# aiven/tiered-storage-for-apache-kafka

Hardware: AMD Instinct MI355X
Metric: GiB/s segment chunk transform (Zstd+AES+CRC), 4MiB chunks (higher is better)
Workload: dtype u8

## Files before the change

### tiered-storage-for-apache-kafka_amd/csrc/crc_dev.h

```cpp
#pragma once
#include "tsx_internal.h"

#define POLY 0x82F63B78u

__host__ __device__ static inline uint32_t crc_mulx(uint32_t v) { return (v >> 1) ^ (POLY & (0u - (v & 1u))); }

__host__ __device__ static inline uint32_t crc_mulmod(uint32_t a, uint32_t b) {
    uint32_t acc = 0;
    for (int i = 0; i < 32; i++) {
        acc ^= b & (0u - ((a >> (31 - i)) & 1u));
        b = crc_mulx(b);
    }
    return acc;
}

__device__ static inline uint32_t crc_pow_pieces(const tsx_crc_tables* tab, uint32_t e) {
    uint32_t r = 0x80000000u;
    for (int k = 0; e; k++, e >>= 1)
        if (e & 1u) r = crc_mulmod(r, tab->pow2[k]);
    return r;
}


__device__ static inline uint32_t crc32c_wave(const tsx_crc_tables* __restrict__ tab, const uint8_t* __restrict__ buf, uint32_t len,
                                              uint32_t* ldsTab, uint32_t lane) {
    {
        const uint4* g = reinterpret_cast<const uint4*>(&tab->slice[0][0]);
        uint4* l = reinterpret_cast<uint4*>(ldsTab);
        for (uint32_t i = lane; i < 4 * 256 / 4; i += 64) l[i] = g[i];
    }
    __syncthreads();
    const uint32_t q = len >> 4;
    const uint32_t per = (((q + 63) >> 6) + 3) & ~3u;
    const uint32_t p0 = min(lane * per, q), p1 = min(p0 + per, q);
    const uint4* in = reinterpret_cast<const uint4*>(buf);
    uint32_t s = 0;
    #define CRC_W(x) { s ^= (x); s = ldsTab[3 * 256 + (s & 0xFF)] ^ ldsTab[2 * 256 + ((s >> 8) & 0xFF)] ^ ldsTab[256 + ((s >> 16) & 0xFF)] ^ ldsTab[s >> 24]; }
    uint32_t p = p0;
    if (p < p1 && p == 0) {
        const uint4 w = in[0];
        CRC_W(w.x ^ 0xFFFFFFFFu) CRC_W(w.y) CRC_W(w.z) CRC_W(w.w)
        p = 1;
    }
    for (; p + 4 <= p1; p += 4) {
        const uint4 w0 = in[p], w1 = in[p + 1], w2 = in[p + 2], w3 = in[p + 3];
        CRC_W(w0.x) CRC_W(w0.y) CRC_W(w0.z) CRC_W(w0.w)
        CRC_W(w1.x) CRC_W(w1.y) CRC_W(w1.z) CRC_W(w1.w)
        CRC_W(w2.x) CRC_W(w2.y) CRC_W(w2.z) CRC_W(w2.w)
        CRC_W(w3.x) CRC_W(w3.y) CRC_W(w3.z) CRC_W(w3.w)
    }
    for (; p < p1; p++) {
        const uint4 w = in[p];
        CRC_W(w.x) CRC_W(w.y) CRC_W(w.z) CRC_W(w.w)
    }
    #undef CRC_W
    uint32_t v = p1 > p0 ? crc_mulmod(s, crc_pow_pieces(tab, q - p1)) : 0u;
    for (int o = 32; o; o >>= 1) v ^= __shfl_xor(v, o);
    if (q == 0) v = 0xFFFFFFFFu;
    const uint8_t* t = buf + ((size_t)q << 4);
    for (uint32_t i = 0; i < (len & 15u); i++) {
        v ^= t[i];
        for (int k = 0; k < 8; k++) v = crc_mulx(v);
    }
    __syncthreads();
    return ~v;
}
```

### tiered-storage-for-apache-kafka_amd/csrc/zstd_enc.hip

```cpp
#include "zstd_common.h"
#ifdef ZS_DBG
#include <stdio.h>
#endif
#include "gcm_dev.h"
#include "crc_dev.h"
#include "svc_dev.h"
#define XXH_WAVE_ATTR __attribute__((noinline))
#include "xxh64_dev.h"

#define LANES 64
#define UNI(x) ((uint32_t)__builtin_amdgcn_readfirstlane((uint32_t)(x)))
#ifdef HIPEMU
#define ZS_GLOBAL
#else
#define ZS_GLOBAL __attribute__((address_space(1)))
#endif
typedef const ZS_GLOBAL uint8_t* gbytes_t;
typedef ZS_GLOBAL uint32_t* gwords_t;
struct __attribute__((packed)) zs_u64u { uint64_t v; };
struct __attribute__((packed)) zs_u32u { uint32_t v; };
__device__ static inline uint64_t gld64(gbytes_t p) { return reinterpret_cast<const ZS_GLOBAL zs_u64u*>(p)->v; }
__device__ static inline uint32_t gld32(gbytes_t p) { return reinterpret_cast<const ZS_GLOBAL zs_u32u*>(p)->v; }
__device__ static inline uint4 ld128a(const uint8_t* p) { return *reinterpret_cast<const uint4*>(p); }
#ifdef HIPEMU
// ... 101 lines not shown
            FseTable of;
            union {
                FseTable ml;
                uint32_t hist[256];
            };
            uint32_t hist2[256];
            uint8_t tableSymbol[512];
            uint16_t cumul[64];
            short norm[64];
        };
        struct {
            uint32_t ring[ZS_RING / 4 + 4];
            uint8_t scr[2 * ZS_SCR];
        } p;
        struct {
            tsx_gf128 tab[256];
            uint32_t t0[256];
        } g;
        uint32_t crcTab[4 * 256];
    };
};

#ifdef HIPEMU
#define WAVE_MEM_SYNC() __threadfence_block()
#define VM_DRAIN() do {} while (0)
#define LOADED64(x) do {} while (0)
#else
#define WAVE_MEM_SYNC() do { asm volatile("" ::: "memory"); __builtin_amdgcn_wave_barrier(); } while (0)
#define VM_DRAIN() asm volatile("s_waitcnt vmcnt(0)" ::: "memory")
#define LOADED64(x) do { uint32_t lo_ = (uint32_t)(x), hi_ = (uint32_t)((x) >> 32); asm volatile("" : "+v"(lo_), "+v"(hi_)); (x) = ((uint64_t)hi_ << 32) | lo_; } while (0)
#endif

struct Win { uint32_t lo, hi; };

__device__ static inline uint64_t ring8(const uint32_t* ring, uint32_t p) {
    uint64_t v; __builtin_memcpy(&v, reinterpret_cast<const uint8_t*>(ring) + (p & (ZS_RING - 1)), 8); return v;
}
__device__ static inline uint32_t ring4(const uint32_t* ring, uint32_t p) {
    uint32_t v; __builtin_memcpy(&v, reinterpret_cast<const uint8_t*>(ring) + (p & (ZS_RING - 1)), 4); return v;
}
__device__ static inline uint32_t ring1(const uint32_t* ring, uint32_t p) { return reinterpret_cast<const uint8_t*>(ring)[p & (ZS_RING - 1)]; }

template <class SP> __device__ __forceinline__ static void win_append(SP src, uint32_t lastPiece, uint32_t* ring, Win& w, uint32_t lane) {
    uint4 v[ZS_FILL / 1024];
    WAVE_MEM_SYNC();
#pragma unroll
    for (uint32_t k = 0; k < ZS_FILL / 1024; k++) {
        uint32_t pp = w.hi + k * 1024 + lane * 16;
        if (pp > lastPiece) pp = lastPiece;
        v[k] = ld128a(src + pp);
// ... 470 lines not shown
                            ip += rl; anchor = ip;
                        }
                    }
                    WAVE_MEM_SYNC();
                    break;
                }
                if (!validm || __builtin_amdgcn_readlane((uint32_t)inPair, 2 * np - 2) == 0) { evType = 4; break; }
                a = __builtin_amdgcn_readlane(la, 2 * np); an = __builtin_amdgcn_readlane(lan, 2 * np);
                s = __builtin_amdgcn_readlane(ls, 2 * np); ns = __builtin_amdgcn_readlane(lns, 2 * np);
                WAVE_MEM_SYNC();
                np = ZS_FAST_PAIRS;
            }
            if (evType == 4) break;
        }
    }
    sav2 = (sav1 != 0 && off1 != 0) ? sav1 : sav2;
    rep[0] = off1 ? off1 : sav1;
    rep[1] = off2 ? off2 : sav2;
    ms.nbSeq = nbSeq; ms.lastLL = iend - anchor; ms.anchor = anchor;
    ms.litSize = litSize + ms.lastLL;
#undef STORE_SEQ
}

__device__ static inline void copy_run(uint8_t* __restrict__ dst, const uint8_t* __restrict__ src, uint32_t n) {
    uint32_t k = 0;
    while (n - k >= 32) {
        const uint64_t a = ld64(src + k), b = ld64(src + k + 8), c = ld64(src + k + 16), d = ld64(src + k + 24);
        __builtin_memcpy(dst + k, &a, 8); __builtin_memcpy(dst + k + 8, &b, 8); __builtin_memcpy(dst + k + 16, &c, 8); __builtin_memcpy(dst + k + 24, &d, 8);
        k += 32;
    }
    const uint32_t r = n - k, nq = r >> 3;
    uint64_t q0 = 0, q1 = 0, q2 = 0; uint32_t w = 0; uint16_t h = 0; uint8_t b1 = 0;
    if (nq > 0) q0 = ld64(src + k);
    if (nq > 1) q1 = ld64(src + k + 8);
    if (nq > 2) q2 = ld64(src + k + 16);
    const uint32_t t = k + 8 * nq;
    if (r & 4) __builtin_memcpy(&w, src + t, 4);
    if (r & 2) __builtin_memcpy(&h, src + t + (r & 4), 2);
    if (r & 1) b1 = src[t + (r & 6)];
    if (nq > 0) __builtin_memcpy(dst + k, &q0, 8);
    if (nq > 1) __builtin_memcpy(dst + k + 8, &q1, 8);
    if (nq > 2) __builtin_memcpy(dst + k + 16, &q2, 8);
    if (r & 4) __builtin_memcpy(dst + t, &w, 4);
    if (r & 2) __builtin_memcpy(dst + t + (r & 4), &h, 2);
    if (r & 1) dst[t + (r & 6)] = b1;
}

__device__ ZS_NOINLINE static void gather_literals(uint8_t* __restrict__ lit, const uint8_t* __restrict__ src, const zs_seq* __restrict__ seqs,
                                                   uint32_t nbSeq, uint32_t tailPos, uint32_t tailLen, uint32_t lane) {
    uint32_t base = 0;
    for (uint32_t g = 0; g < nbSeq; g += LANES) {
        const uint32_t u = g + lane;
        uint32_t ll = 0, lp = 0;
        if (u < nbSeq) { const zs_seq q = seqs[u]; ll = q.litLength; lp = q.litPos; }
        uint32_t incl = ll;
        for (int o = 1; o < LANES; o <<= 1) { const uint32_t t = __shfl_up(incl, o); if (lane >= (uint32_t)o) incl += t; }
        const uint32_t dst = base + incl - ll;
        copy_run(lit + dst, src + lp, ll);
        base += __shfl(incl, LANES - 1);
    }
    for (uint32_t i = lane; i < tailLen; i += LANES) lit[base + i] = src[tailPos + i];
}

struct BitW { uint8_t* start; uint8_t* p; uint8_t* end; uint64_t acc; uint32_t n; bool overflow; };
__device__ static inline void bw_init(BitW& b, uint8_t* dst, uint8_t* end) { b.start = b.p = dst; b.end = end; b.acc = 0; b.n = 0; b.overflow = false; }
__device__ static inline void bw_add(BitW& b, uint64_t v, uint32_t nb) {
    if (!nb) return;
    b.acc |= (v & ((1ull << nb) - 1)) << b.n;
    b.n += nb;
    while (b.n >= 8) { if (b.p < b.end) *b.p++ = (uint8_t)b.acc; else b.overflow = true; b.acc >>= 8; b.n -= 8; }
}
__device__ static inline uint32_t bw_close(BitW& b) {
    bw_add(b, 1, 1);
    if (b.n) { if (b.p < b.end) *b.p++ = (uint8_t)b.acc; else b.overflow = true; b.n = 0; }
    return (uint32_t)(b.p - b.start);
}

__device__ static uint32_t fse_minTableLog(uint32_t srcSize, uint32_t maxSym) {
    uint32_t a = hb32(srcSize) + 1, b = hb32(maxSym) + 2;
    return a < b ? a : b;
}
__device__ static uint32_t fse_optimalTableLog(uint32_t maxTableLog, uint32_t srcSize, uint32_t maxSym, uint32_t minus) {
    uint32_t maxBitsSrc = hb32(srcSize - 1) - minus, tableLog = maxTableLog, minBits = fse_minTableLog(srcSize, maxSym);
    if (maxBitsSrc < tableLog) tableLog = maxBitsSrc;
// ... 430 lines not shown
                }
            }
        }
    }
    if ((hSize > 1) & (hSize < maxSym / 2)) { dst[0] = (uint8_t)hSize; return hSize + 1; }
    if (maxSym > 128) return 0xFFFFFFFFu;
    dst[0] = (uint8_t)(128 + (maxSym - 1));
    hw[maxSym] = 0;
    for (uint32_t n = 0; n < maxSym; n += 2) dst[(n / 2) + 1] = (uint8_t)((hw[n] << 4) + hw[n + 1]);
    return ((maxSym + 1) / 2) + 1;
}

__device__ static inline uint32_t wave_sum(uint32_t v) { for (int o = 32; o; o >>= 1) v += __shfl_xor(v, o); return v; }
__device__ static inline uint32_t wave_max(uint32_t v) { for (int o = 32; o; o >>= 1) { uint32_t t = __shfl_xor(v, o); v = t > v ? t : v; } return v; }
__device__ static inline uint32_t wave_excl_scan(uint32_t v, uint32_t lane) {
    uint32_t s = v;
    for (int o = 1; o < LANES; o <<= 1) { uint32_t t = __shfl_up(s, o); if (lane >= (uint32_t)o) s += t; }
    return s - v;
}

__device__ ZS_NOINLINE static void wave_histogram(uint32_t* hist, const uint8_t* __restrict__ p, uint32_t n, uint32_t lane) {
    for (uint32_t i = lane; i < 256; i += LANES) hist[i] = 0;
    __syncthreads();
    for (uint32_t i = lane; i < n; i += LANES) atomicAdd(&hist[p[i]], 1u);
    __syncthreads();
}

__device__ ZS_NOINLINE static uint32_t wave_huf_encode(uint32_t* __restrict__ tmp, const uint8_t* __restrict__ src, uint32_t n, const HufTable& ct, uint32_t lane) {
    const uint32_t per = (n + LANES - 1) / LANES;
    const uint32_t r0 = lane * per < n ? lane * per : n, r1 = r0 + per < n ? r0 + per : n;
    uint32_t bits = 0;
    for (uint32_t r = r0; r < r1; r++) bits += ct.nb[src[n - 1 - r]];
    const uint32_t startBit = wave_excl_scan(bits, lane);
    const uint32_t total = __shfl(startBit + bits, LANES - 1);
    const uint32_t words = (total + 1 + 31) / 32;
    for (uint32_t w = lane; w < words; w += LANES) tmp[w] = 0;
    __threadfence_block();
    __syncthreads();
    {   uint64_t acc = 0; uint32_t word = startBit >> 5, nacc = startBit & 31;
        for (uint32_t r = r0; r < r1; r++) {
            const uint8_t s = src[n - 1 - r];
            acc |= (uint64_t)ct.val[s] << nacc;
            nacc += ct.nb[s];
            if (nacc >= 32) { atomicOr(&tmp[word], (uint32_t)acc); acc >>= 32; nacc -= 32; word++; }
        }
        if (lane == LANES - 1) { acc |= 1ull << nacc; nacc++; }
        if (nacc) atomicOr(&tmp[word], (uint32_t)acc);
        if (nacc > 32) atomicOr(&tmp[word + 1], (uint32_t)(acc >> 32));
    }
    __threadfence_block();
    __syncthreads();
    return (total + 1 + 7) / 8;
}

__device__ static inline void wave_copy(uint8_t* __restrict__ dst, const uint8_t* __restrict__ src, uint32_t n, uint32_t lane) {
    for (uint32_t i = lane; i < n; i += LANES) dst[i] = src[i];
}

__device__ ZS_NOINLINE static uint32_t wave_huf_compress(uint8_t* ostart, uint8_t* op, const uint8_t* __restrict__ lit, uint32_t n, bool single, const HufTable& ct,
                                             uint32_t* tmp, uint32_t lane) {
    if (single) {
        const uint32_t c = wave_huf_encode(tmp, lit, n, ct, lane);
        wave_copy(op, (const uint8_t*)tmp, c, lane);
        op += c;
    } else {
        if (n < 12) return 0;
        const uint32_t seg = (n + 3) / 4;
        uint8_t* const jump = op;
        op += 6;
        for (int i = 0; i < 4; i++) {
            const uint32_t len = i < 3 ? seg : n - 3 * seg;
            const uint32_t c = wave_huf_encode(tmp, lit + (uint32_t)i * seg, len, ct, lane);
            if (c == 0 || c > 65535) return 0;
            if (i < 3 && lane == 0) { jump[2 * i] = (uint8_t)c; jump[2 * i + 1] = (uint8_t)(c >> 8); }
            wave_copy(op, (const uint8_t*)tmp, c, lane);
            op += c;
            __syncthreads();
        }
    }
    const uint32_t tot = (uint32_t)(op - ostart);
    if (tot >= n - 1) return 0;
    return tot;
}

__device__ static uint32_t write_raw_literals(uint8_t* dst, const uint8_t* lit, uint32_t n, uint32_t lane) {
    const uint32_t fl = 1 + (n > 31) + (n > 4095);
    WAVE_MEM_SYNC();
    if (lane == 0) {
        if (fl == 1) dst[0] = (uint8_t)(0 + (n << 3));
        else if (fl == 2) { const uint32_t v = 0 + (1 << 2) + (n << 4); dst[0] = (uint8_t)v; dst[1] = (uint8_t)(v >> 8); }
        else { const uint32_t v = 0 + (3 << 2) + (n << 4); dst[0] = (uint8_t)v; dst[1] = (uint8_t)(v >> 8); dst[2] = (uint8_t)(v >> 16); }
    }
    wave_copy(dst + fl, lit, n, lane);
    return fl + n;
}
__device__ static uint32_t write_rle_literals(uint8_t* dst, const uint8_t* lit, uint32_t n, uint32_t lane) {
    const uint32_t fl = 1 + (n > 31) + (n > 4095);
    WAVE_MEM_SYNC();
    if (lane == 0) {
        if (fl == 1) dst[0] = (uint8_t)(1 + (n << 3));
        else if (fl == 2) { const uint32_t v = 1 + (1 << 2) + (n << 4); dst[0] = (uint8_t)v; dst[1] = (uint8_t)(v >> 8); }
        else { const uint32_t v = 1 + (3 << 2) + (n << 4); dst[0] = (uint8_t)v; dst[1] = (uint8_t)(v >> 8); dst[2] = (uint8_t)(v >> 16); }
        dst[fl] = lit[0];
    }
    return fl + 1;
}

__device__ ZS_NOINLINE static uint32_t compress_literals(uint8_t* dst, const uint8_t* __restrict__ lit, uint32_t n, EncLds& L, int cur, bool suspectUncompressible,
                                             uint32_t* tmp, uint32_t lane) {
    const int nxt = cur ^ 1;
    const uint32_t lhSize = 3 + (n >= 1024) + (n >= 16384);
    bool single = n < 256;
    if (n < 64) return write_raw_literals(dst, lit, n, lane);
    const int prevRepeat = L.hufRepeat[cur];
    const bool preferRepeat = n <= 1024;
    uint8_t* const ostart = dst + lhSize;
    uint32_t cLit = 0; bool usedOld = false, newTable = false;
    bool decided = false;
    if (suspectUncompressible && n >= 40960) {
        wave_histogram(L.hist2, lit, 4096, lane);
        uint32_t m = 0; for (uint32_t i = lane; i < 256; i += LANES) m = L.hist2[i] > m ? L.hist2[i] : m;
        uint32_t largestTotal = wave_max(m);
        __syncthreads();
        wave_histogram(L.hist2, lit + n - 4096, 4096, lane);
        m = 0; for (uint32_t i = lane; i < 256; i += LANES) m = L.hist2[i] > m ? L.hist2[i] : m;
        largestTotal += wave_max(m);
        if (largestTotal <= ((2 * 4096) >> 7) + 4) { cLit = 0; decided = true; }
    }
    uint32_t maxSym = 255, largest = 0;
    if (!decided) {
        PT(5);
        wave_histogram(L.hist, lit, n, lane);
        uint32_t m = 0, top = 0;
        for (uint32_t i = lane; i < 256; i += LANES) { const uint32_t c = L.hist[i]; if (c > m) m = c; if (c) top = i; }
        largest = wave_max(m); maxSym = wave_max(top);
        if (largest == n) { cLit = 1; decided = true; if (lane == 0) ostart[0] = lit[0]; }
        else if (largest <= (n >> 7) + 4) { cLit = 0; decided = true; }
    }
    if (!decided) {
        int repeat = prevRepeat;
        if (repeat == 1) {
            bool bad = L.huf[cur].maxSym < maxSym;
            for (uint32_t i = lane; i <= maxSym; i += LANES) bad |= (L.hist[i] != 0) & (L.huf[cur].nb[i] == 0);
            if (__any(bad)) repeat = 0;
        }
        if (preferRepeat && repeat != 0) {
            cLit = wave_huf_compress(ostart, ostart, lit, n, single, L.huf[cur], tmp, lane);
            usedOld = true;
        } else {
            PT(5);
            static_assert(sizeof(L.of) >= HUF_WORK_A_BYTES, "the first group of work arrays fits the OF table");
            static_assert(offsetof(EncLds, norm) + sizeof(((EncLds*)0)->norm) - (offsetof(EncLds, hist) + sizeof(((EncLds*)0)->hist)) >= HUF_WORK_B_BYTES && (offsetof(EncLds, hist) & 3) == 0,
                          "lcount[-1 .. 255] + par[512] fit behind the byte histogram");
            uint32_t huffLog = fse_optimalTableLog(ZS_LitHufLog, n, maxSym, 1);
            huffLog = UNI(huf_buildCTable(L.huf[nxt], L.hist, maxSym, huffLog, reinterpret_cast<uint8_t*>(&L.of), reinterpret_cast<uint8_t*>(L.hist) + sizeof(L.hist), &L.scal[4], lane));
            uint32_t oldBits = 0, newBits = 0;
            if (repeat != 0) {
                for (uint32_t s_ = lane; s_ <= maxSym; s_ += LANES) { oldBits += L.huf[cur].nb[s_] * L.hist[s_]; newBits += L.huf[nxt].nb[s_] * L.hist[s_]; }
                oldBits = wave_sum(oldBits); newBits = wave_sum(newBits);
            }
            if (lane == 0) {
                const uint32_t hSize = huf_writeCTable(ostart, L.huf[nxt], maxSym, huffLog, L);
                uint32_t useOld = 0, fail = 0;
                if (hSize == 0xFFFFFFFFu) fail = 1;
                else {
                    if (repeat != 0) {
                        if ((oldBits >> 3) <= hSize + (newBits >> 3) || hSize + 12 >= n) useOld = 1;
                    }
                    if (!useOld && hSize + 12 >= n) fail = 1;
                }
                L.scal[0] = hSize; L.scal[1] = useOld; L.scal[2] = fail;
            }
            __syncthreads();
            const uint32_t hSize = L.scal[0]; const bool useOld = L.scal[1], fail = L.scal[2];
            __syncthreads();
            PT(6);
            if (fail) cLit = 0;
            else if (useOld) { cLit = wave_huf_compress(ostart, ostart, lit, n, single, L.huf[cur], tmp, lane); usedOld = true; }
            else { cLit = wave_huf_compress(ostart, ostart + hSize, lit, n, single, L.huf[nxt], tmp, lane); newTable = true; }
        }
    }
    PT(7);
    const uint32_t minGain = (n >> 6) + 2;
    if (cLit == 0 || cLit >= n - minGain) return write_raw_literals(dst, lit, n, lane);
    if (cLit == 1) return write_rle_literals(dst, lit, n, lane);
    const uint32_t hType = (usedOld && !newTable) ? 3u : 2u;
    if (newTable) L.scal[8] = 1;
    if (lane == 0) {
        if (lhSize == 3) { const uint32_t v = hType + ((uint32_t)(!single) << 2) + (n << 4) + (cLit << 14); dst[0] = (uint8_t)v; dst[1] = (uint8_t)(v >> 8); dst[2] = (uint8_t)(v >> 16); }
        else if (lhSize == 4) { const uint32_t v = hType + (2 << 2) + (n << 4) + (cLit << 18); dst[0] = (uint8_t)v; dst[1] = (uint8_t)(v >> 8); dst[2] = (uint8_t)(v >> 16); dst[3] = (uint8_t)(v >> 24); }
        else { const uint32_t v = hType + (3 << 2) + (n << 4) + (cLit << 22); dst[0] = (uint8_t)v; dst[1] = (uint8_t)(v >> 8); dst[2] = (uint8_t)(v >> 16); dst[3] = (uint8_t)(v >> 24); dst[4] = (uint8_t)(cLit >> 10); }
    }
    return lhSize + cLit;
}

__device__ static int select_encoding(uint32_t mostFrequent, uint32_t nbSeq, uint32_t defaultNormLog, bool defaultAllowed, uint32_t mult) {
    if (mostFrequent == nbSeq) return (defaultAllowed && nbSeq <= 2) ? 0 : 1;
    if (defaultAllowed) {
        const uint32_t dynMin = ((1u << defaultNormLog) * mult) >> 3;
        if (nbSeq < dynMin || mostFrequent < (nbSeq >> (defaultNormLog - 1))) return 0;
    }
    return 2;
// ... 7 lines not shown
    for (uint32_t s = 0; s <= max; s++) if (cnt[s] > mostFrequent) mostFrequent = cnt[s];
    const bool defaultAllowed = isOffsets ? (max <= ZS_DefaultMaxOff) : true;
    const int t = select_encoding(mostFrequent, nbSeq, defaultNormLog, defaultAllowed, L.scal[ZS_SCAL_MULT]);
    *type = (uint32_t)t;
    if (t == 1) {
        ct.tableLog = 0; ct.state[0] = 0; ct.state[1] = 0; ct.dnb[max] = 0; ct.dfs[max] = 0;
        *op = codes[0];
        return 1;
    }
    if (t == 0) {
        for (uint32_t s = 0; s <= defaultMax; s++) L.norm[s] = defaultNorm[s];
        fse_buildCTable(ct, L.norm, defaultMax, defaultNormLog, L.cumul, L.tableSymbol);
        return 0;
    }
    uint32_t nbSeq_1 = nbSeq;
    const uint32_t tableLog = fse_optimalTableLog(FSELog, nbSeq, max, 2);
    if (cnt[codes[nbSeq - 1]] > 1) { cnt[codes[nbSeq - 1]]--; nbSeq_1--; }
    if (fse_normalizeCount(L.norm, tableLog, cnt, nbSeq_1, max, nbSeq_1 >= 2048) < 0) return 0xFFFFFFFFu;
    const uint32_t sz = fse_writeNCount(op, L.norm, max, tableLog);
    fse_buildCTable(ct, L.norm, max, tableLog, L.cumul, L.tableSymbol);
    return sz;
}

__device__ ZS_NOINLINE static uint32_t compress_sequences(uint8_t* op0, uint8_t* oend, const zs_seq* __restrict__ seqs, uint32_t nbSeq, uint8_t* __restrict__ codes,
                                              EncLds& L, uint32_t* tmp, uint32_t tmpCap, uint32_t lane) {
    uint8_t* op = op0;
    uint8_t* const llC = codes; uint8_t* const ofC = codes + ZS_WS_CODE_STRIDE; uint8_t* const mlC = codes + 2 * ZS_WS_CODE_STRIDE;
    if (lane == 0) {
        if (nbSeq < 128) *op = (uint8_t)nbSeq;
        else if (nbSeq < 0x7F00) { op[0] = (uint8_t)((nbSeq >> 8) + 0x80); op[1] = (uint8_t)nbSeq; }
        else { op[0] = 0xFF; op[1] = (uint8_t)(nbSeq - 0x7F00); op[2] = (uint8_t)((nbSeq - 0x7F00) >> 8); }
    }
    op += nbSeq < 128 ? 1 : nbSeq < 0x7F00 ? 2 : 3;
    if (nbSeq == 0) return (uint32_t)(op - op0);
    uint32_t* const cLL = L.hist2; uint32_t* const cOF = L.hist2 + 64; uint32_t* const cML = L.hist2 + 128;
    for (uint32_t i = lane; i < 192; i += LANES) L.hist2[i] = 0;
    __syncthreads();
    for (uint32_t u = lane; u < nbSeq; u += LANES) {
        const zs_seq q = seqs[u];
        const uint32_t a = LLcode(q.litLength), b = hb32(q.offBase), c = MLcode(q.mlBase);
        llC[u] = (uint8_t)a; ofC[u] = (uint8_t)b; mlC[u] = (uint8_t)c;
        atomicAdd(&cLL[a], 1u); atomicAdd(&cOF[b], 1u); atomicAdd(&cML[c], 1u);
    }
    __threadfence_block();
    __syncthreads();
    PT(8);
    if (lane == 0) {
        uint8_t* const seqHead = op; uint8_t* q = op + 1;
// ... 37 lines not shown
                for (int j = 7; j >= 0; j--) {
                    if (j <= top) {
                        const uint32_t nb = (st + dn[j]) >> 16;
                        ob[j >> 1] |= ((st & ((1u << nb) - 1)) | (nb << 12)) << (16 * (j & 1));
                        st = ct.state[(st >> nb) + df[j]];
                    }
                }
                if (top == 7) *reinterpret_cast<uint4*>(o + g) = make_uint4(ob[0], ob[1], ob[2], ob[3]);
                else {
#pragma unroll
                    for (int j = 0; j < 8; j++) if (j <= top) o[g + j] = (uint16_t)(ob[j >> 1] >> (16 * (j & 1)));
                }
                if (g == 0) break;
                g -= 8; n = (int32_t)g + 7; cur = nxt;
            }
        }
        finalState = st & ((1u << ct.tableLog) - 1); finalLog = ct.tableLog;
    }
    __threadfence_block();
    __syncthreads();
    PT(10);
    const uint32_t fLL = __shfl(finalState, 0), fOF = __shfl(finalState, 1), fML = __shfl(finalState, 2);
    const uint32_t gLL = __shfl(finalLog, 0), gOF = __shfl(finalLog, 1), gML = __shfl(finalLog, 2);
    const uint32_t per = (nbSeq + LANES - 1) / LANES;
    const uint32_t r0 = lane * per < nbSeq ? lane * per : nbSeq, r1 = r0 + per < nbSeq ? r0 + per : nbSeq;
    uint32_t bits = 0;
    for (uint32_t r = r0; r < r1; r++) {
        const uint32_t n = nbSeq - 1 - r;
        bits += (stb[n] >> 12) + (stb[ZS_WS_CODE_STRIDE + n] >> 12) + (stb[2 * ZS_WS_CODE_STRIDE + n] >> 12) + kLLbits[llC[n]] + kMLbits[mlC[n]] + ofC[n];
    }
    if (lane == LANES - 1) bits += gML + gOF + gLL + 1;
    const uint32_t startBit = wave_excl_scan(bits, lane);
    const uint32_t totalBits = __shfl(startBit + bits, LANES - 1);
    const uint32_t bitstreamSize = (totalBits + 7) / 8;
    uint8_t* const q = op0 + qoff;
    if (q + bitstreamSize > oend || bitstreamSize > tmpCap) return 0xFFFFFFFFu;
    {   const uint32_t words = (totalBits + 31) / 32 + 1;
        for (uint32_t wd = lane; wd < words; wd += LANES) tmp[wd] = 0;
    }
    __threadfence_block();
    __syncthreads();
    {   uint64_t acc = 0; uint32_t word = startBit >> 5, nacc = startBit & 31;
#define SEQ_PUT(v, nb) do { acc |= (uint64_t)(v) << nacc; nacc += (nb); if (nacc >= 32) { atomicOr(&tmp[word], (uint32_t)acc); acc >>= 32; nacc -= 32; word++; } } while (0)
        for (uint32_t r = r0; r < r1; r++) {
            const uint32_t n = nbSeq - 1 - r;
            const zs_seq sq = seqs[n];
            const uint32_t lc = llC[n], oc = ofC[n], mc = mlC[n];
            const uint32_t sLL = stb[n], sOF = stb[ZS_WS_CODE_STRIDE + n], sML = stb[2 * ZS_WS_CODE_STRIDE + n];
            const uint32_t nOF = sOF >> 12, nML = sML >> 12, nLL = sLL >> 12;
            const uint32_t v1 = (sOF & 0xFFF) | ((sML & 0xFFF) << nOF) | ((sLL & 0xFFF) << (nOF + nML));
            SEQ_PUT(v1, nOF + nML + nLL);
            const uint32_t bl = kLLbits[lc], bm = kMLbits[mc];
            const uint64_t v2 = (uint64_t)(sq.litLength & ((1u << bl) - 1)) | ((uint64_t)(sq.mlBase & ((1u << bm) - 1)) << bl);
            SEQ_PUT(v2, bl + bm);
            SEQ_PUT(sq.offBase & (uint32_t)((1ull << oc) - 1), oc);
        }
        if (lane == LANES - 1) {
            SEQ_PUT(fML, gML); SEQ_PUT(fOF, gOF); SEQ_PUT(fLL, gLL);
            SEQ_PUT(1u, 1u);
        }
#undef SEQ_PUT
        if (nacc) atomicOr(&tmp[word], (uint32_t)acc);
    }
    __threadfence_block();
    __syncthreads();
    wave_copy(q, (const uint8_t*)tmp, bitstreamSize, lane);
    __threadfence_block();
    __syncthreads();
    PT(10);
    if (lastCountSize && (lastCountSize + bitstreamSize) < 4) return 0xFFFFFFFFu;
    return qoff + bitstreamSize;
}

__device__ ZS_NOINLINE static uint32_t split_block_1_5_7(const uint8_t* __restrict__ p, EncLds& L, uint32_t lane) {
    uint32_t* past = L.hist; uint32_t* cur = L.hist2;
    uint32_t pastN = 0; int penalty = 3;
    for (uint32_t i = lane; i < 256; i += LANES) past[i] = 0;
    __syncthreads();
    for (uint32_t n = lane * 43; n < 8191; n += LANES * 43) atomicAdd(&past[p[n]], 1u);
    pastN = 8191 / 43;
    __syncthreads();
    for (uint32_t pos = 8192; pos <= ZS_BLOCK_MAX - 8192; pos += 8192) {
        for (uint32_t i = lane; i < 256; i += LANES) cur[i] = 0;
        __syncthreads();
        for (uint32_t n = lane * 43; n < 8191; n += LANES * 43) atomicAdd(&cur[p[pos + n]], 1u);
        const uint32_t curN = 8191 / 43;
        __syncthreads();
        uint64_t dev = 0;
        for (uint32_t i = lane; i < 256; i += LANES) {
// ... 108 lines not shown
                                                           int32_t* __restrict__ status, uint8_t* __restrict__ work, uint32_t profile, uint32_t level_word, uint32_t sched,
                                                           const tsx_chain_fuse fuse, const uint32_t chunk, const svc_handback hb
#ifdef TSX_PROF
                                                           , unsigned long long* __restrict__ prof_out
#endif
                                                           ) {
    const uint32_t lane = threadIdx.x;
    const uint32_t level = level_word & ~TSX_ZSEG_CHECKSUM;
    const bool checksum = (level_word & TSX_ZSEG_CHECKSUM) != 0;
#ifdef TSX_PROF
    if (lane == 0) { for (int i = 0; i < 24; i++) g_prof[i] = 0; g_prof[22] = g_prof[23] = (unsigned long long)clock64(); g_prof[2] = wall_clock64(); }
    __syncthreads();
#endif
    const uint8_t* __restrict__ src = src_base + descs[chunk].src_off;
    const uint32_t srcSize = descs[chunk].src_len;
    uint8_t* const frame = mid + (uint64_t)chunk * mid_stride;
    uint8_t* const ws = work + (size_t)chunk * ZS_WS_BYTES;
    uint32_t* const hashLong = (uint32_t*)(ws + ZS_WS_HASHLONG);
    uint32_t* const hashSmall = (uint32_t*)(ws + ZS_WS_HASHSMALL);
    zs_seq* const seqs = (zs_seq*)(ws + ZS_WS_SEQS);
    uint8_t* const lit = ws + ZS_WS_LIT;
    uint8_t* const codes = ws + ZS_WS_CODES;
    uint8_t* const blockout = ws + ZS_WS_BLOCKOUT;
    uint32_t* const huftmp = (uint32_t*)(blockout + (256u << 10));
    if (fuse.crc) {
        const uint32_t crc = crc32c_wave(fuse.crc, src, srcSize, L.crcTab, lane);
        if (lane == 0) descs[chunk].crc32c = crc;
        PT(16);
    }
    if (fuse.self_status) { if (lane == 0) status[chunk] = TSX_OK; }
    else if (status[chunk] != TSX_OK) { if (lane == 0) { zlen[chunk] = 0; if (fuse.key) descs[chunk].dst_len = 0; } return false; }

    zs_cparams cp = zs_level3_cparams(srcSize);
    bool fast = false;
    if (level == 1 || level == 2) {
        const zs_level_params q = zs_level_cparams((int)level, srcSize ? srcSize : 1);
        cp.windowLog = q.windowLog; cp.chainLog = q.chainLog; cp.hashLog = q.hashLog; cp.minMatch = q.minMatch;
        fast = q.strategy == ZS_STRAT_FAST;
    }
    {
        uint4 z; z.x = z.y = z.z = z.w = 0;
        uint4* a = (uint4*)hashLong; uint4* b = (uint4*)hashSmall;
        for (uint32_t i = lane; i < (1u << cp.hashLog) / 4; i += LANES) a[i] = z;
        if (!fast) for (uint32_t i = lane; i < (1u << cp.chainLog) / 4; i += LANES) b[i] = z;
    }
    uint32_t hdr = 0;
    {   const uint32_t windowSize = 1u << cp.windowLog;
// ... 45 lines not shown
        const uint32_t lastBlock = blockSize == remaining;
        {
            const uint32_t blockEndIdx = ipos + 2, maxDist = 1u << cp.windowLog;
            if (blockEndIdx > maxDist && dictLimit < blockEndIdx - maxDist) dictLimit = blockEndIdx - maxDist;
        }
        uint32_t cSize = 0;
        if (blockSize >= 7) {
            uint32_t rep[3] = {repc[0], repc[1], repc[2]};
            MfState ms;
            if (fast) fast_block(src, ipos, blockSize, hashLong, cp, dictLimit, rep, seqs, ms, L.p.ring, lane);
            else match_block(src, srcSize, ipos, blockSize, hashLong, hashSmall, cp, dictLimit, rep, seqs, ms, L.p.ring, L.p.scr, lane, sched);
            __threadfence_block();
            __syncthreads();
            gather_literals(lit, src, seqs, ms.nbSeq, ms.anchor, ms.lastLL, lane);
            __threadfence_block();
            __syncthreads();
            PT(18); PCNT(20, 1);
            if (lane == 0) L.scal[8] = 0;
            __syncthreads();
            const bool suspect = ms.nbSeq == 0 || (ms.litSize / ms.nbSeq >= 20);
            for (uint32_t i = lane; i < sizeof(L.huf) / 4; i += LANES) reinterpret_cast<uint32_t*>(&L.huf[0])[i] = hufSave[i];
            __threadfence_block();
            __syncthreads();
            uint32_t litBytes = UNI(compress_literals(blockout, lit, ms.litSize, L, cur, suspect, huftmp, lane));
            __threadfence_block();
            __syncthreads();
            for (uint32_t i = lane; i < sizeof(L.huf) / 4; i += LANES) hufSave[i] = reinterpret_cast<const uint32_t*>(&L.huf[0])[i];
            __threadfence_block();
            __syncthreads();
            uint32_t seqBytes = UNI(compress_sequences(blockout + litBytes, blockout + (255u << 10), seqs, ms.nbSeq, codes, L, huftmp, (ZS_BLOCKOUT_CAP - (256u << 10)) - 64, lane));
            const bool newHuf = UNI(L.scal[8]) != 0;
            if (seqBytes != 0xFFFFFFFFu) {
                cSize = litBytes + seqBytes;
                const uint32_t maxCSize = blockSize - ((blockSize >> 6) + 2);
                if (cSize >= maxCSize) cSize = 0;
            }
            if (!first && ms.nbSeq < 4 && ms.litSize < 10 && wave_is_rle(src + ipos, blockSize, lane)) cSize = 1;
            if (cSize > 1) {
                repc[0] = rep[0]; repc[1] = rep[1]; repc[2] = rep[2];
                if (newHuf) { cur ^= 1; if (lane == 0) L.hufRepeat[cur] = 1; }
                __syncthreads();
            }
        }
        if (cSize == 0) {
            if (lane == 0) { const uint32_t h = lastBlock + (0u << 1) + (blockSize << 3); op[0] = (uint8_t)h; op[1] = (uint8_t)(h >> 8); op[2] = (uint8_t)(h >> 16); }
            wave_copy(op + 3, src + ipos, blockSize, lane);
            cSize = 3 + blockSize;
        } else if (cSize == 1) {
            if (lane == 0) { const uint32_t h = lastBlock + (1u << 1) + (blockSize << 3); op[0] = (uint8_t)h; op[1] = (uint8_t)(h >> 8); op[2] = (uint8_t)(h >> 16); op[3] = src[ipos]; }
            cSize = 4;
        } else {
            if (lane == 0) { const uint32_t h = lastBlock + (2u << 1) + (cSize << 3); op[0] = (uint8_t)h; op[1] = (uint8_t)(h >> 8); op[2] = (uint8_t)(h >> 16); }
            wave_copy(op + 3, blockout, cSize, lane);
// ... 133 lines not shown
```

Measured before the change: 19.80.

## Encode Huffman and sequence bitstreams in place, vectorize copies, histogram and prefetch loads

Huffman encoding now writes straight into the output buffer. Lanes own whole interior words and only boundary words use atomics, which removes the global temp buffer and the extra copy. Sequence encoding is reworked to process 64 sequences per step, scatter bits into a small LDS staging area and stream finished words out with a carry, again dropping the temp buffer and copy. Smaller pieces come along with it: a 16-byte vectorized wave_copy with an alignment head, a histogram that reads uint4 words, software prefetch in the CRC and literal-gather loops, and double-buffered loads. The cost is more barriers per sequence group and more complex bit-boundary handling, which adds correctness risk.

```diff
diff --git a/tiered-storage-for-apache-kafka_amd/csrc/crc_dev.h b/tiered-storage-for-apache-kafka_amd/csrc/crc_dev.h
--- a/tiered-storage-for-apache-kafka_amd/csrc/crc_dev.h
+++ b/tiered-storage-for-apache-kafka_amd/csrc/crc_dev.h
@@ -42,12 +42,16 @@
         CRC_W(w.x ^ 0xFFFFFFFFu) CRC_W(w.y) CRC_W(w.z) CRC_W(w.w)
         p = 1;
     }
-    for (; p + 4 <= p1; p += 4) {
-        const uint4 w0 = in[p], w1 = in[p + 1], w2 = in[p + 2], w3 = in[p + 3];
-        CRC_W(w0.x) CRC_W(w0.y) CRC_W(w0.z) CRC_W(w0.w)
-        CRC_W(w1.x) CRC_W(w1.y) CRC_W(w1.z) CRC_W(w1.w)
-        CRC_W(w2.x) CRC_W(w2.y) CRC_W(w2.z) CRC_W(w2.w)
-        CRC_W(w3.x) CRC_W(w3.y) CRC_W(w3.z) CRC_W(w3.w)
+    if (p + 4 <= p1) {
+        uint4 n0 = in[p], n1 = in[p + 1], n2 = in[p + 2], n3 = in[p + 3];
+        for (; p + 4 <= p1; p += 4) {
+            const uint4 w0 = n0, w1 = n1, w2 = n2, w3 = n3;
+            if (p + 8 <= p1) { n0 = in[p + 4]; n1 = in[p + 5]; n2 = in[p + 6]; n3 = in[p + 7]; }
+            CRC_W(w0.x) CRC_W(w0.y) CRC_W(w0.z) CRC_W(w0.w)
+            CRC_W(w1.x) CRC_W(w1.y) CRC_W(w1.z) CRC_W(w1.w)
+            CRC_W(w2.x) CRC_W(w2.y) CRC_W(w2.z) CRC_W(w2.w)
+            CRC_W(w3.x) CRC_W(w3.y) CRC_W(w3.z) CRC_W(w3.w)
+        }
     }
     for (; p < p1; p++) {
         const uint4 w = in[p];
diff --git a/tiered-storage-for-apache-kafka_amd/csrc/zstd_enc.hip b/tiered-storage-for-apache-kafka_amd/csrc/zstd_enc.hip
--- a/tiered-storage-for-apache-kafka_amd/csrc/zstd_enc.hip
+++ b/tiered-storage-for-apache-kafka_amd/csrc/zstd_enc.hip
@@ -147,10 +147,12 @@
 };
 
 #ifdef HIPEMU
+__device__ static inline void zs_atomic_and(uint32_t* p, uint32_t v) { *p &= v; }
 #define WAVE_MEM_SYNC() __threadfence_block()
 #define VM_DRAIN() do {} while (0)
 #define LOADED64(x) do {} while (0)
 #else
+__device__ static inline void zs_atomic_and(uint32_t* p, uint32_t v) { atomicAnd(p, v); }
 #define WAVE_MEM_SYNC() do { asm volatile("" ::: "memory"); __builtin_amdgcn_wave_barrier(); } while (0)
 #define VM_DRAIN() asm volatile("s_waitcnt vmcnt(0)" ::: "memory")
 #define LOADED64(x) do { uint32_t lo_ = (uint32_t)(x), hi_ = (uint32_t)((x) >> 32); asm volatile("" : "+v"(lo_), "+v"(hi_)); (x) = ((uint64_t)hi_ << 32) | lo_; } while (0)
@@ -667,6 +669,23 @@
 #undef STORE_SEQ
 }
 
+__device__ ZS_NOINLINE static void wave_copy(uint8_t* __restrict__ dst, const uint8_t* __restrict__ src, uint32_t n, uint32_t lane) {
+    uint32_t head = (uint32_t)((0 - (uintptr_t)dst) & 15);
+    if (head > n) head = n;
+    if (lane < head) dst[lane] = src[lane];
+    const uint32_t q = (n - head) >> 4;
+    uint8_t* const d = dst + head; const uint8_t* const s = src + head;
+    uint32_t i = lane;
+    for (; i + 3 * LANES < q; i += 4 * LANES) {
+        const uint4 v0 = ld128(s + 16 * i), v1 = ld128(s + 16 * (i + LANES)), v2 = ld128(s + 16 * (i + 2 * LANES)), v3 = ld128(s + 16 * (i + 3 * LANES));
+        *reinterpret_cast<uint4*>(d + 16 * i) = v0; *reinterpret_cast<uint4*>(d + 16 * (i + LANES)) = v1;
+        *reinterpret_cast<uint4*>(d + 16 * (i + 2 * LANES)) = v2; *reinterpret_cast<uint4*>(d + 16 * (i + 3 * LANES)) = v3;
+    }
+    for (; i < q; i += LANES) *reinterpret_cast<uint4*>(d + 16 * i) = ld128(s + 16 * i);
+    const uint32_t t = head + (q << 4) + lane;
+    if (t < n) dst[t] = src[t];
+}
+
 __device__ static inline void copy_run(uint8_t* __restrict__ dst, const uint8_t* __restrict__ src, uint32_t n) {
     uint32_t k = 0;
     while (n - k >= 32) {
@@ -694,17 +713,20 @@
 __device__ ZS_NOINLINE static void gather_literals(uint8_t* __restrict__ lit, const uint8_t* __restrict__ src, const zs_seq* __restrict__ seqs,
                                                    uint32_t nbSeq, uint32_t tailPos, uint32_t tailLen, uint32_t lane) {
     uint32_t base = 0;
+    uint32_t nll = 0, nlp = 0;
+    if (lane < nbSeq) { const zs_seq q = seqs[lane]; nll = q.litLength; nlp = q.litPos; }
     for (uint32_t g = 0; g < nbSeq; g += LANES) {
-        const uint32_t u = g + lane;
-        uint32_t ll = 0, lp = 0;
-        if (u < nbSeq) { const zs_seq q = seqs[u]; ll = q.litLength; lp = q.litPos; }
+        const uint32_t ll = nll, lp = nlp;
+        const uint32_t u = g + LANES + lane;
+        nll = 0; nlp = 0;
+        if (u < nbSeq) { const zs_seq q = seqs[u]; nll = q.litLength; nlp = q.litPos; }
         uint32_t incl = ll;
         for (int o = 1; o < LANES; o <<= 1) { const uint32_t t = __shfl_up(incl, o); if (lane >= (uint32_t)o) incl += t; }
         const uint32_t dst = base + incl - ll;
         copy_run(lit + dst, src + lp, ll);
         base += __shfl(incl, LANES - 1);
     }
-    for (uint32_t i = lane; i < tailLen; i += LANES) lit[base + i] = src[tailPos + i];
+    wave_copy(lit + base, src + tailPos, tailLen, lane);
 }
 
 struct BitW { uint8_t* start; uint8_t* p; uint8_t* end; uint64_t acc; uint32_t n; bool overflow; };
@@ -1181,47 +1203,82 @@
 __device__ ZS_NOINLINE static void wave_histogram(uint32_t* hist, const uint8_t* __restrict__ p, uint32_t n, uint32_t lane) {
     for (uint32_t i = lane; i < 256; i += LANES) hist[i] = 0;
     __syncthreads();
-    for (uint32_t i = lane; i < n; i += LANES) atomicAdd(&hist[p[i]], 1u);
-    __syncthreads();
-}
-
-__device__ ZS_NOINLINE static uint32_t wave_huf_encode(uint32_t* __restrict__ tmp, const uint8_t* __restrict__ src, uint32_t n, const HufTable& ct, uint32_t lane) {
-    const uint32_t per = (n + LANES - 1) / LANES;
+    const uint32_t q = n >> 4;
+    for (uint32_t i = lane; i < q; i += LANES) {
+        const uint4 v = ld128(p + 16 * i);
+        const uint32_t w[4] = {v.x, v.y, v.z, v.w};
+#pragma unroll
+        for (int k = 0; k < 4; k++) {
+            atomicAdd(&hist[w[k] & 0xFF], 1u); atomicAdd(&hist[(w[k] >> 8) & 0xFF], 1u);
+            atomicAdd(&hist[(w[k] >> 16) & 0xFF], 1u); atomicAdd(&hist[w[k] >> 24], 1u);
+        }
+    }
+    for (uint32_t i = (q << 4) + lane; i < n; i += LANES) atomicAdd(&hist[p[i]], 1u);
+    __syncthreads();
+}
+
+#define HUF_SYMS16(v, OP) do { const uint32_t w_[4] = {(v).x, (v).y, (v).z, (v).w}; \
+        _Pragma("unroll") for (int k_ = 3; k_ >= 0; k_--) { OP(w_[k_] >> 24) OP((w_[k_] >> 16) & 0xFF) OP((w_[k_] >> 8) & 0xFF) OP(w_[k_] & 0xFF) } } while (0)
+__device__ ZS_NOINLINE static uint32_t wave_huf_encode(uint8_t* __restrict__ dst, const uint8_t* __restrict__ src, uint32_t n, const HufTable& ct, uint32_t lane) {
+    const uint32_t per = ((n + LANES - 1) / LANES + 15) & ~15u;
     const uint32_t r0 = lane * per < n ? lane * per : n, r1 = r0 + per < n ? r0 + per : n;
+    const uint32_t a = n - r1, b = n - r0;
     uint32_t bits = 0;
-    for (uint32_t r = r0; r < r1; r++) bits += ct.nb[src[n - 1 - r]];
-    const uint32_t startBit = wave_excl_scan(bits, lane);
-    const uint32_t total = __shfl(startBit + bits, LANES - 1);
-    const uint32_t words = (total + 1 + 31) / 32;
-    for (uint32_t w = lane; w < words; w += LANES) tmp[w] = 0;
+    {   uint32_t e = b;
+        uint4 nxt = make_uint4(0, 0, 0, 0);
+        if (e - a >= 16) nxt = ld128(src + e - 16);
+        while (e - a >= 16) {
+            const uint4 v = nxt;
+            e -= 16;
+            if (e - a >= 16) nxt = ld128(src + e - 16);
+#define HUF_CNT(s_) bits += ct.nb[s_];
+            HUF_SYMS16(v, HUF_CNT);
+#undef HUF_CNT
+        }
+        while (e > a) bits += ct.nb[src[--e]];
+    }
+    if (lane == LANES - 1) bits += 1;
+    const uint32_t shift = 8 * (uint32_t)((uintptr_t)dst & 3);
+    uint32_t* const wbase = reinterpret_cast<uint32_t*>(dst - (shift >> 3));
+    const uint32_t startBit = shift + wave_excl_scan(bits, lane);
+    const uint32_t endBit = __shfl(startBit + bits, LANES - 1);
+    VM_DRAIN();
+    if (bits) {
+        const uint32_t w0 = startBit >> 5, w1 = (startBit + bits - 1) >> 5;
+        if (w0 == 0 && shift) zs_atomic_and(&wbase[0], (1u << shift) - 1); else wbase[w0] = 0;
+        if (w1 != w0) wbase[w1] = 0;
+    }
     __threadfence_block();
     __syncthreads();
     {   uint64_t acc = 0; uint32_t word = startBit >> 5, nacc = startBit & 31;
-        for (uint32_t r = r0; r < r1; r++) {
-            const uint8_t s = src[n - 1 - r];
-            acc |= (uint64_t)ct.val[s] << nacc;
-            nacc += ct.nb[s];
-            if (nacc >= 32) { atomicOr(&tmp[word], (uint32_t)acc); acc >>= 32; nacc -= 32; word++; }
-        }
-        if (lane == LANES - 1) { acc |= 1ull << nacc; nacc++; }
-        if (nacc) atomicOr(&tmp[word], (uint32_t)acc);
-        if (nacc > 32) atomicOr(&tmp[word + 1], (uint32_t)(acc >> 32));
+        bool shared = true;
+#define HUF_FLUSH() do { if (shared) { atomicOr(&wbase[word], (uint32_t)acc); shared = false; } else wbase[word] = (uint32_t)acc; acc >>= 32; nacc -= 32; word++; } while (0)
+#define HUF_PUT(s_) { const uint32_t sy_ = (s_); acc |= (uint64_t)ct.val[sy_] << nacc; nacc += ct.nb[sy_]; if (nacc >= 32) HUF_FLUSH(); }
+        uint32_t e = b;
+        uint4 nxt = make_uint4(0, 0, 0, 0);
+        if (e - a >= 16) nxt = ld128(src + e - 16);
+        while (e - a >= 16) {
+            const uint4 v = nxt;
+            e -= 16;
+            if (e - a >= 16) nxt = ld128(src + e - 16);
+            HUF_SYMS16(v, HUF_PUT);
+        }
+        while (e > a) HUF_PUT(src[--e])
+        if (lane == LANES - 1) { acc |= 1ull << nacc; nacc++; if (nacc >= 32) HUF_FLUSH(); }
+        if (nacc && acc) atomicOr(&wbase[word], (uint32_t)acc);
+#undef HUF_PUT
+#undef HUF_FLUSH
     }
     __threadfence_block();
     __syncthreads();
-    return (total + 1 + 7) / 8;
-}
-
-__device__ static inline void wave_copy(uint8_t* __restrict__ dst, const uint8_t* __restrict__ src, uint32_t n, uint32_t lane) {
-    for (uint32_t i = lane; i < n; i += LANES) dst[i] = src[i];
-}
+    return (endBit - shift + 7) / 8;
+}
+#undef HUF_SYMS16
 
 __device__ ZS_NOINLINE static uint32_t wave_huf_compress(uint8_t* ostart, uint8_t* op, const uint8_t* __restrict__ lit, uint32_t n, bool single, const HufTable& ct,
-                                             uint32_t* tmp, uint32_t lane) {
+                                             uint32_t lane) {
     if (single) {
-        const uint32_t c = wave_huf_encode(tmp, lit, n, ct, lane);
-        wave_copy(op, (const uint8_t*)tmp, c, lane);
-        op += c;
+        op += wave_huf_encode(op, lit, n, ct, lane);
     } else {
         if (n < 12) return 0;
         const uint32_t seg = (n + 3) / 4;
@@ -1229,10 +1286,9 @@
         op += 6;
         for (int i = 0; i < 4; i++) {
             const uint32_t len = i < 3 ? seg : n - 3 * seg;
-            const uint32_t c = wave_huf_encode(tmp, lit + (uint32_t)i * seg, len, ct, lane);
+            const uint32_t c = wave_huf_encode(op, lit + (uint32_t)i * seg, len, ct, lane);
             if (c == 0 || c > 65535) return 0;
             if (i < 3 && lane == 0) { jump[2 * i] = (uint8_t)c; jump[2 * i + 1] = (uint8_t)(c >> 8); }
-            wave_copy(op, (const uint8_t*)tmp, c, lane);
             op += c;
             __syncthreads();
         }
@@ -1266,7 +1322,7 @@
 }
 
 __device__ ZS_NOINLINE static uint32_t compress_literals(uint8_t* dst, const uint8_t* __restrict__ lit, uint32_t n, EncLds& L, int cur, bool suspectUncompressible,
-                                             uint32_t* tmp, uint32_t lane) {
+                                             uint32_t lane) {
     const int nxt = cur ^ 1;
     const uint32_t lhSize = 3 + (n >= 1024) + (n >= 16384);
     bool single = n < 256;
@@ -1304,7 +1360,7 @@
             if (__any(bad)) repeat = 0;
         }
         if (preferRepeat && repeat != 0) {
-            cLit = wave_huf_compress(ostart, ostart, lit, n, single, L.huf[cur], tmp, lane);
+            cLit = wave_huf_compress(ostart, ostart, lit, n, single, L.huf[cur], lane);
             usedOld = true;
         } else {
             PT(5);
@@ -1335,8 +1391,8 @@
             __syncthreads();
             PT(6);
             if (fail) cLit = 0;
-            else if (useOld) { cLit = wave_huf_compress(ostart, ostart, lit, n, single, L.huf[cur], tmp, lane); usedOld = true; }
-            else { cLit = wave_huf_compress(ostart, ostart + hSize, lit, n, single, L.huf[nxt], tmp, lane); newTable = true; }
+            else if (useOld) { cLit = wave_huf_compress(ostart, ostart, lit, n, single, L.huf[cur], lane); usedOld = true; }
+            else { cLit = wave_huf_compress(ostart, ostart + hSize, lit, n, single, L.huf[nxt], lane); newTable = true; }
         }
     }
     PT(7);
@@ -1390,8 +1446,21 @@
     return sz;
 }
 
+struct SeqIn { uint32_t ll, ml, ob, lc, oc, mc, sLL, sOF, sML; };
+__device__ static inline SeqIn seq_load(const zs_seq* __restrict__ seqs, const uint8_t* __restrict__ codes, const uint16_t* __restrict__ stb, uint32_t nbSeq, uint32_t r) {
+    SeqIn in = {0, 0, 0, 0, 0, 0, 0, 0, 0};
+    if (r < nbSeq) {
+        const uint32_t n = nbSeq - 1 - r;
+        const zs_seq sq = seqs[n];
+        in.ll = sq.litLength; in.ml = sq.mlBase; in.ob = sq.offBase;
+        in.lc = codes[n]; in.oc = codes[ZS_WS_CODE_STRIDE + n]; in.mc = codes[2 * ZS_WS_CODE_STRIDE + n];
+        in.sLL = stb[n]; in.sOF = stb[ZS_WS_CODE_STRIDE + n]; in.sML = stb[2 * ZS_WS_CODE_STRIDE + n];
+    }
+    return in;
+}
+
 __device__ ZS_NOINLINE static uint32_t compress_sequences(uint8_t* op0, uint8_t* oend, const zs_seq* __restrict__ seqs, uint32_t nbSeq, uint8_t* __restrict__ codes,
-                                              EncLds& L, uint32_t* tmp, uint32_t tmpCap, uint32_t lane) {
+                                              EncLds& L, uint32_t cap, uint32_t lane) {
     uint8_t* op = op0;
     uint8_t* const llC = codes; uint8_t* const ofC = codes + ZS_WS_CODE_STRIDE; uint8_t* const mlC = codes + 2 * ZS_WS_CODE_STRIDE;
     if (lane == 0) {
@@ -1475,49 +1544,62 @@
     PT(10);
     const uint32_t fLL = __shfl(finalState, 0), fOF = __shfl(finalState, 1), fML = __shfl(finalState, 2);
     const uint32_t gLL = __shfl(finalLog, 0), gOF = __shfl(finalLog, 1), gML = __shfl(finalLog, 2);
-    const uint32_t per = (nbSeq + LANES - 1) / LANES;
-    const uint32_t r0 = lane * per < nbSeq ? lane * per : nbSeq, r1 = r0 + per < nbSeq ? r0 + per : nbSeq;
-    uint32_t bits = 0;
-    for (uint32_t r = r0; r < r1; r++) {
-        const uint32_t n = nbSeq - 1 - r;
-        bits += (stb[n] >> 12) + (stb[ZS_WS_CODE_STRIDE + n] >> 12) + (stb[2 * ZS_WS_CODE_STRIDE + n] >> 12) + kLLbits[llC[n]] + kMLbits[mlC[n]] + ofC[n];
-    }
-    if (lane == LANES - 1) bits += gML + gOF + gLL + 1;
-    const uint32_t startBit = wave_excl_scan(bits, lane);
-    const uint32_t totalBits = __shfl(startBit + bits, LANES - 1);
+    uint8_t* const q = op0 + qoff;
+    if (q > oend) return 0xFFFFFFFFu;
+    const uint32_t capBytes = (uint32_t)(oend - q) < cap ? (uint32_t)(oend - q) : cap;
+    const uint32_t shift = 8 * (uint32_t)((uintptr_t)q & 3);
+    uint32_t* const wbase = reinterpret_cast<uint32_t*>(q - (shift >> 3));
+    uint32_t* const sb = L.hist2;
+    static_assert(sizeof(L.hist2) >= 4 * (179 + 3), "one step of sequence bits fits the dead histogram");
+    uint32_t carry = shift ? wbase[0] & ((1u << shift) - 1) : 0u, carryN = shift;
+    uint32_t wordsDone = 0, totalBits = 0;
+    SeqIn nx = seq_load(seqs, codes, stb, nbSeq, lane);
+    for (uint32_t g = 0; g < nbSeq; g += LANES) {
+        const SeqIn in = nx;
+        if (g + LANES < nbSeq) nx = seq_load(seqs, codes, stb, nbSeq, g + LANES + lane);
+        const uint32_t nOF = in.sOF >> 12, nML = in.sML >> 12, nLL = in.sLL >> 12;
+        const uint32_t v1 = (in.sOF & 0xFFF) | ((in.sML & 0xFFF) << nOF) | ((in.sLL & 0xFFF) << (nOF + nML));
+        const uint32_t bl = kLLbits[in.lc], bm = kMLbits[in.mc], nb1 = nOF + nML + nLL;
+        const uint64_t v2 = (uint64_t)(in.ll & ((1u << bl) - 1)) | ((uint64_t)(in.ml & ((1u << bm) - 1)) << bl);
+        const uint64_t v12 = (uint64_t)v1 | (v2 << nb1);
+        const uint32_t nb12 = nb1 + bl + bm;
+        const uint32_t v3 = in.ob & (uint32_t)((1ull << in.oc) - 1);
+        const uint32_t bits = g + lane < nbSeq ? nb12 + in.oc : 0u;
+        const uint32_t off = carryN + wave_excl_scan(bits, lane);
+        const uint32_t groupEnd = __shfl(off + bits, LANES - 1);
+        totalBits += groupEnd - carryN;
+        if (totalBits > 8 * capBytes) return 0xFFFFFFFFu;
+        for (uint32_t i = lane; i < ((groupEnd + 31) >> 5) + 3; i += LANES) sb[i] = i ? 0u : carry;
+        __syncthreads();
+        if (bits) {
+            const uint32_t w = off >> 5, sh = off & 31;
+            const uint64_t lo = v12 << sh;
+            const uint32_t hi = sh ? (uint32_t)(v12 >> (64 - sh)) : 0u;
+            if ((uint32_t)lo) atomicOr(&sb[w], (uint32_t)lo);
+            if ((uint32_t)(lo >> 32)) atomicOr(&sb[w + 1], (uint32_t)(lo >> 32));
+            if (hi) atomicOr(&sb[w + 2], hi);
+            const uint32_t off3 = off + nb12, w3 = off3 >> 5;
+            const uint64_t t = (uint64_t)v3 << (off3 & 31);
+            if ((uint32_t)t) atomicOr(&sb[w3], (uint32_t)t);
+            if ((uint32_t)(t >> 32)) atomicOr(&sb[w3 + 1], (uint32_t)(t >> 32));
+        }
+        __syncthreads();
+        const uint32_t full = groupEnd >> 5;
+        for (uint32_t i = lane; i < full; i += LANES) wbase[wordsDone + i] = sb[i];
+        carry = sb[full]; carryN = groupEnd & 31;
+        wordsDone += full;
+        __syncthreads();
+    }
+    {
+        const uint32_t nbF = gML + gOF + gLL + 1;
+        const uint64_t vF = (uint64_t)fML | ((uint64_t)fOF << gML) | ((uint64_t)fLL << (gML + gOF)) | (1ull << (gML + gOF + gLL));
+        totalBits += nbF;
+        if (totalBits > 8 * capBytes) return 0xFFFFFFFFu;
+        const uint64_t t = (uint64_t)carry | (vF << carryN);
+        uint8_t* const e = reinterpret_cast<uint8_t*>(wbase + wordsDone);
+        if (lane < (carryN + nbF + 7) / 8) e[lane] = (uint8_t)(t >> (8 * lane));
+    }
     const uint32_t bitstreamSize = (totalBits + 7) / 8;
-    uint8_t* const q = op0 + qoff;
-    if (q + bitstreamSize > oend || bitstreamSize > tmpCap) return 0xFFFFFFFFu;
-    {   const uint32_t words = (totalBits + 31) / 32 + 1;
-        for (uint32_t wd = lane; wd < words; wd += LANES) tmp[wd] = 0;
-    }
-    __threadfence_block();
-    __syncthreads();
-    {   uint64_t acc = 0; uint32_t word = startBit >> 5, nacc = startBit & 31;
-#define SEQ_PUT(v, nb) do { acc |= (uint64_t)(v) << nacc; nacc += (nb); if (nacc >= 32) { atomicOr(&tmp[word], (uint32_t)acc); acc >>= 32; nacc -= 32; word++; } } while (0)
-        for (uint32_t r = r0; r < r1; r++) {
-            const uint32_t n = nbSeq - 1 - r;
-            const zs_seq sq = seqs[n];
-            const uint32_t lc = llC[n], oc = ofC[n], mc = mlC[n];
-            const uint32_t sLL = stb[n], sOF = stb[ZS_WS_CODE_STRIDE + n], sML = stb[2 * ZS_WS_CODE_STRIDE + n];
-            const uint32_t nOF = sOF >> 12, nML = sML >> 12, nLL = sLL >> 12;
-            const uint32_t v1 = (sOF & 0xFFF) | ((sML & 0xFFF) << nOF) | ((sLL & 0xFFF) << (nOF + nML));
-            SEQ_PUT(v1, nOF + nML + nLL);
-            const uint32_t bl = kLLbits[lc], bm = kMLbits[mc];
-            const uint64_t v2 = (uint64_t)(sq.litLength & ((1u << bl) - 1)) | ((uint64_t)(sq.mlBase & ((1u << bm) - 1)) << bl);
-            SEQ_PUT(v2, bl + bm);
-            SEQ_PUT(sq.offBase & (uint32_t)((1ull << oc) - 1), oc);
-        }
-        if (lane == LANES - 1) {
-            SEQ_PUT(fML, gML); SEQ_PUT(fOF, gOF); SEQ_PUT(fLL, gLL);
-            SEQ_PUT(1u, 1u);
-        }
-#undef SEQ_PUT
-        if (nacc) atomicOr(&tmp[word], (uint32_t)acc);
-    }
-    __threadfence_block();
-    __syncthreads();
-    wave_copy(q, (const uint8_t*)tmp, bitstreamSize, lane);
     __threadfence_block();
     __syncthreads();
     PT(10);
@@ -1672,7 +1754,6 @@
     uint8_t* const lit = ws + ZS_WS_LIT;
     uint8_t* const codes = ws + ZS_WS_CODES;
     uint8_t* const blockout = ws + ZS_WS_BLOCKOUT;
-    uint32_t* const huftmp = (uint32_t*)(blockout + (256u << 10));
     if (fuse.crc) {
         const uint32_t crc = crc32c_wave(fuse.crc, src, srcSize, L.crcTab, lane);
         if (lane == 0) descs[chunk].crc32c = crc;
@@ -1764,13 +1845,13 @@
             for (uint32_t i = lane; i < sizeof(L.huf) / 4; i += LANES) reinterpret_cast<uint32_t*>(&L.huf[0])[i] = hufSave[i];
             __threadfence_block();
             __syncthreads();
-            uint32_t litBytes = UNI(compress_literals(blockout, lit, ms.litSize, L, cur, suspect, huftmp, lane));
+            uint32_t litBytes = UNI(compress_literals(blockout, lit, ms.litSize, L, cur, suspect, lane));
             __threadfence_block();
             __syncthreads();
             for (uint32_t i = lane; i < sizeof(L.huf) / 4; i += LANES) hufSave[i] = reinterpret_cast<const uint32_t*>(&L.huf[0])[i];
             __threadfence_block();
             __syncthreads();
-            uint32_t seqBytes = UNI(compress_sequences(blockout + litBytes, blockout + (255u << 10), seqs, ms.nbSeq, codes, L, huftmp, (ZS_BLOCKOUT_CAP - (256u << 10)) - 64, lane));
+            uint32_t seqBytes = UNI(compress_sequences(blockout + litBytes, blockout + (255u << 10), seqs, ms.nbSeq, codes, L, (ZS_BLOCKOUT_CAP - (256u << 10)) - 64, lane));
             const bool newHuf = UNI(L.scal[8]) != 0;
             if (seqBytes != 0xFFFFFFFFu) {
                 cSize = litBytes + seqBytes;
```

Measured after the change: 21.42 (median of 6 runs). +8.2%, better.
